# wuji3/visiondk

Hardware: AMD Instinct MI355X
Metric: images/sec fwd+bwd+optimizer step (ViT-B/16, bs=256 per GPU) (higher is better)
Workload: dtype fp16; 1 GPU; ViT-B/16 ICT, synthetic ImageNet-1k 224x224, random-init weights (reference re-init), per-GPU batch 256, CE label_smoothing 0.05, SGD 0.006/0.937/5e-4, clip 10, EMA on rank 0; global_batch=256, parallelism=dp1

## Files before the change

visiondk_amd/csrc/vit_engine.hip:

```cpp
#include <hip/hip_runtime.h>
#include <stdlib.h>
#include <stdio.h>
#include <string.h>
#include "vdk_device.h"
#include "vdk_host.h"
#include "vdk_gemm.h"

extern "C" {
int vdk_layernorm_fwd(const float*, int64_t, int32_t, int32_t, const float*, const float*, float, void*, int64_t, int32_t, float*, float*, void*);
int vdk_layernorm_bwd_workspace_bytes(int32_t, int32_t, size_t*);
int vdk_layernorm_bwd(const void*, int64_t, int32_t, const float*, int64_t, const float*, const float*, const float*, const float*, int64_t,
                      int32_t, int32_t, float*, int64_t, void*, int64_t, float*, float*, void*, size_t, void*);
int vdk_reduce_rows_f32(const float*, int64_t, int32_t, int64_t, float*, float, void*);
int vdk_colsum_bf16_workspace_bytes(int32_t, int32_t, size_t*);
int vdk_colsum_bf16(const void*, int64_t, int32_t, int32_t, float*, void*, size_t, void*);
int vdk_attention_fwd(const void*, int64_t, void*, int64_t, float*, int32_t, int32_t, int32_t, int32_t, float, void*);
int vdk_attention_bwd(const void*, int64_t, const void*, const void*, int64_t, const float*, void*, int64_t, float*, int32_t, int32_t, int32_t,
                      int32_t, float, void*);
int vdk_attention_fwd_dt(const void*, int64_t, void*, int64_t, float*, int32_t, int32_t, int32_t, int32_t, float, int32_t, void*);
int vdk_attention_bwd_dt(const void*, int64_t, const void*, const void*, int64_t, const float*, void*, int64_t, float*, int32_t, int32_t, int32_t, int32_t, float, int32_t, void*);
int vdk_attention_bwd_cs(const void*, int64_t, const void*, const void*, int64_t, const float*, void*, int64_t, float*, int32_t, int32_t, int32_t, int32_t, float, int32_t, float*, int32_t*,
                         void*);
int vdk_patchify_bf16(const float*, int32_t, int32_t, int32_t, int32_t, int32_t, void*, int32_t, void*);
int vdk_cls_rows(float*, int64_t, int32_t, int32_t, const float*, const float*, void*);
// ... 161 lines not shown
  size_t dxa, dxm;
  size_t dxab[3], dxmb[2];
  size_t du[2], dqkv[2];
  size_t dsm;
  size_t dvec;
  size_t tA, tB;
  size_t slabs, slabs_bytes;
  size_t lnws, lnws_bytes, csws, csws_bytes;
  size_t dhf;
  size_t dposall;
  size_t a8;
  size_t a8b;
};
static size_t w_take(size_t& cur, size_t n) { size_t o = cur; cur = (cur + n + 255) & ~(size_t)255; return o; }
static int wgrad_splitk(int M, int N, int K) {
  if (K < 4096) return 1;
  int tiles = ((M + 127) / 128) * ((N + 127) / 128);
  int s = (1024 + tiles - 1) / tiles;
  if (s > 32) s = 32;
  if (s < 1) s = 1;
  return s;
}
static int wgrad_splitk_tn(int M, int N, int K) {
  const int tiles = ((M + 255) / 256) * ((N + 255) / 256);
  int s = 256 / tiles;
  if (s < 1) s = 1;
  const int kt = K / 64;
  if (s > kt / 4) s = kt / 4;
  if (s > 64) s = 64;
  if (s < 1) s = 1;
  return s;
}
static int vit_plan(const VitDims& d, WsPlan* w) {
  size_t cur = 0;
  const size_t T = d.T, D = d.D, M = d.M, L = d.L;
  w->patches = w_take(cur, (size_t)d.B * d.np * d.Kpe * 2);
  w->pepad = w->dwpe = 0;
  if (d.Kraw != d.Kpe) { w->pepad = w_take(cur, D * d.Kpe * 2); w->dwpe = w_take(cur, D * d.Kpe * 4); }
  w->X = w_take(cur, (2 * L + 1) * T * D * 4);
  w->xe = w->pstats = 0;
  if (d.pre) { w->xe = w_take(cur, T * D * 4); w->pstats = w_take(cur, 2 * T * 4); }
  w->stats = w_take(cur, (L * 4 * T + 2 * T) * 4);
  w->s_h = T * D * 2; w->s_qkv = T * 3 * D * 2; w->s_lse = (size_t)d.B * d.H * d.N * 4; w->s_u = T * M * 2;
  w->h1 = w_take(cur, L * w->s_h); w->qkv = w_take(cur, L * w->s_qkv); w->lse = w_take(cur, L * w->s_lse);
  w->o = w_take(cur, L * w->s_h); w->h2 = w_take(cur, L * w->s_h); w->u = w_take(cur, L * w->s_u); w->g = w_take(cur, L * w->s_u);
  w->hf = w_take(cur, (size_t)d.Bp * D * 2);
  w->dxa = w_take(cur, T * D * 4); w->dxm = w_take(cur, T * D * 4);
  size_t big = M > 3 * D ? M : 3 * D;
  for (int i = 0; i < 3; ++i) w->dxab[i] = w_take(cur, T * D * 2);
  for (int i = 0; i < 2; ++i) {
    w->dxmb[i] = w_take(cur, T * D * 2);
    w->du[i] = w_take(cur, T * M * 2); w->dqkv[i] = w_take(cur, T * 3 * D * 2);
  }
  w->dsm = w_take(cur, T * D * 2);
  w->dvec = w_take(cur, w->s_lse);
  size_t trows = big > (size_t)d.Cp ? big : (size_t)d.Cp;
  if (trows < (size_t)d.Kpe) trows = d.Kpe;
  size_t tcols = d.Tp > d.Bp ? d.Tp : d.Bp;
  w->tA = w_take(cur, trows * tcols * 2); w->tB = w_take(cur, trows * tcols * 2);
  size_t sl = 0;
  {
    int sh[5][3] = {{(int)M, (int)D, d.T}, {(int)D, (int)M, d.T}, {3 * (int)D, (int)D, d.T}, {(int)D, (int)D, d.T}, {(int)D, d.Kpe, d.B * d.np}};
    for (auto& s : sh) {
      int k1 = wgrad_splitk(s[0], s[1], s[2]), k2 = wgrad_splitk_tn(s[0], s[1], s[2]);
      size_t b = (size_t)(k1 > k2 ? k1 : k2) * s[0] * s[1] * 4; if (b > sl) sl = b;
    }
  }
  w->slabs_bytes = sl; w->slabs = w_take(cur, sl);
  vdk_layernorm_bwd_workspace_bytes(d.T, d.D, &w->lnws_bytes); w->lnws_bytes = (w->lnws_bytes + 255) & ~(size_t)255; w->lnws = w_take(cur, 2 * w->lnws_bytes);
  size_t cs = (size_t)((tcols + 63) / 64) * trows * 4;
  { size_t cs2 = 0; vdk_colsum_bf16_workspace_bytes(d.T, (int)trows, &cs2); if (cs2 > cs) cs = cs2; }
  { size_t cs3 = (size_t)2 * ((d.T + 255) / 256) * trows * 4; if (cs3 > cs) cs = cs3; }
  w->csws_bytes = (cs + 255) & ~(size_t)255; w->csws = w_take(cur, 5 * w->csws_bytes);
  w->dhf = w_take(cur, (size_t)d.B * D * 2);
  w->dposall = w_take(cur, (size_t)d.N * D * 4);
  w->a8 = d.fp8 ? w_take(cur, T * (M > 3 * D ? M : 3 * D)) : 0;
  w->a8b = d.fp8 ? w_take(cur, T * M) : 0;
  w->total = cur;
  return VDK_OK;
}

#define RC(x) do { int rc_ = (x); if (rc_) return rc_; } while (0)

struct F8 {
  int mode; unsigned char* w8; unsigned char* wt8; float* amax; float* sc; float* si; unsigned char* a8; unsigned char* a8b;
};
static int f8_init(const VdkVitConfig* cfg, const VitDims& d, const PLayout& p, F8* f, unsigned char* a8, unsigned char* a8b) {
  f->mode = d.fp8; f->a8 = a8; f->a8b = a8b;
  if (!d.fp8) return VDK_OK;
  if (!cfg->fp8_w || !cfg->fp8_state) return vdk_fail(VDK_EINVAL, "vit: fp8 mode without fp8_w / fp8_state");
  if (a8 && d.T < 256) return vdk_fail(VDK_EUNSUPPORTED, "vit: the fp8 mode needs batch * tokens >= 256");
  f->w8 = (unsigned char*)cfg->fp8_w; f->wt8 = f->w8 + p.total;
  const int S = 12 * d.L;
  f->amax = cfg->fp8_state; f->sc = f->amax + S; f->si = f->sc + S;
  return VDK_OK;
}
static int f8_quant(hipStream_t s, const F8& f, const void* x, int xdt, long n, int slot, int fmt, unsigned char* out, int force_current = 0) {
  if (f.mode == 2 || force_current) {
    RC(vdk_quant_fp8(x, xdt, n, nullptr, nullptr, fmt, f.amax + slot, s));
    RC(vdk_fp8_scale_update(f.amax + slot, f.sc + slot, f.si + slot, 1, fmt, 1.0f, s));
  }
  return vdk_quant_fp8(x, xdt, n, f.sc + slot, out, fmt, f.amax + slot, s);
}
static bool f8_fused(const F8& f) {
  const char* e = getenv("VDK_FP8_FUSED_QUANT");
  return f.mode == 1 && !(e && e[0] == '0');
}
static int gemm8(hipStream_t s, const F8& f, const void* a, int slot_a, int a_fmt, const unsigned char* w8, int slot_w, int64_t ldb, void* Cc, int64_t ldc, int M, int N,
                 int K, int cdt, const float* bias, const float* res, int64_t ldr, int act, void* aux, int64_t ldaux, const unsigned char* a_pre = nullptr, int q8_slot = -1,
                 int q8_fmt = 0, float* c_colsum = nullptr) {
  if (!a_pre) RC(f8_quant(s, f, a, VDK_BF16, (long)M * K, slot_a, a_fmt, f.a8));
  VdkGemmDesc g = {};
  g.A = a_pre ? a_pre : f.a8; g.lda = K; g.B = w8; g.ldb = ldb; g.C = Cc; g.ldc = ldc; g.M = M; g.N = N; g.K = K; g.c_dtype = cdt; g.bias = bias; g.residual = res; g.ldr = ldr;
  g.act = act; g.aux = aux; g.ldaux = ldaux; g.alpha = 1.0f; g.splitk = 1; g.c_colsum = c_colsum;
  if (q8_slot >= 0) return vdk_gemm_fp8_nt_q8(&g, a_fmt, 0, f.si + slot_a, f.si + slot_w, f.a8b, N, q8_fmt, f.sc + q8_slot, f.amax + q8_slot, s);
  return vdk_gemm_fp8_nt(&g, a_fmt, 0, f.si + slot_a, f.si + slot_w, s);
}
__global__ void vit_fp8_update_kernel(float* __restrict__ amax, float* __restrict__ sc, float* __restrict__ si, int n) {
  const int i = blockIdx.x * blockDim.x + threadIdx.x;
  if (i >= n) return;
  const float a = amax[i], fmax = (i % 12) >= 8 ? 57344.0f : 448.0f;
  if (a > 0.f && a < 3.0e38f) { const float v = fmax / a; sc[i] = v; si[i] = 1.0f / v; }
  amax[i] = 0.f;
}

#include <map>
#include <vector>
static thread_local std::map<int, std::vector<hipEvent_t>> g_ev_dev;
static int ev_get(size_t i, hipEvent_t* e) {
  int dev = 0; (void)hipGetDevice(&dev);
  std::vector<hipEvent_t>& g_ev = g_ev_dev[dev];
  while (g_ev.size() <= i) {
    hipEvent_t x;
    if (hipEventCreateWithFlags(&x, hipEventDisableTiming) != hipSuccess) return vdk_fail(VDK_ELAUNCH, "vit: hipEventCreate failed");
    g_ev.push_back(x);
  }
  *e = g_ev[i];
  return VDK_OK;
}
static int ev_order(size_t slot, hipStream_t from, hipStream_t to) {
  if (from == to) return VDK_OK;
  hipEvent_t e; RC(ev_get(slot, &e));
  if (hipEventRecord(e, from) != hipSuccess || hipStreamWaitEvent(to, e, 0) != hipSuccess) return vdk_fail(VDK_ELAUNCH, "vit: event record/wait failed");
  return VDK_OK;
}

static int gemm(hipStream_t s, const void* A, int64_t lda, const void* B, int64_t ldb, void* C, int64_t ldc, int M, int N, int K, int cdt,
                const float* bias, const float* res, int64_t ldr, int act, void* aux, int64_t ldaux, int splitk, int row_group, void* ws,
                size_t wsb) {
  VdkGemmDesc g = {};
  g.A = A; g.lda = lda; g.B = B; g.ldb = ldb; g.C = C; g.ldc = ldc; g.M = M; g.N = N; g.K = K; g.c_dtype = cdt == VDK_F32 ? VDK_F32 : DT16; g.bias = bias;
  g.residual = res; g.ldr = ldr; g.act = act; g.aux = aux; g.ldaux = ldaux; g.alpha = 1.0f; g.splitk = splitk; g.row_group = row_group; g.ab_dtype = DT16;
  return vdk_gemm_bf16_nt(&g, ws, wsb, s);
}

extern "C" {

int vdk_vit_param_count(const VdkVitConfig* cfg, int64_t* n_floats, int32_t* n_tensors, int64_t* n_transposed) {
  VitDims d; RC(vit_dims(cfg, &d));
  PLayout p; RC(vit_layout(d, &p));
  if (n_floats) *n_floats = p.total;
  if (n_tensors) *n_tensors = 3 + d.pre + d.cls + 12 * d.L + (d.C > 0 ? 4 : 2);
  if (n_transposed) *n_transposed = p.totalT;
  return VDK_OK;
}

// ... 15 lines not shown
  VitDims d; RC(vit_dims(cfg, &d));
  WsPlan w; RC(vit_plan(d, &w));
  if (!bytes) return vdk_fail(VDK_EINVAL, "null");
  *bytes = w.total;
  return VDK_OK;
}

int vdk_vit_refresh_weights(const VdkVitConfig* cfg, const float* params, void* wb16, void* wt16, int32_t skip_wb16, void* stream) {
  VitDims d; RC(vit_dims(cfg, &d));
  PLayout p; RC(vit_layout(d, &p));
  if (!params || !wb16 || !wt16) return vdk_fail(VDK_EINVAL, "vdk_vit_refresh_weights: null pointer");
  t_opf = d.opf;
  if (!skip_wb16) RC(vdk_cast_f32_16(params, wb16, p.total, t_opf, stream));
  bf16_t* wt = (bf16_t*)wt16;
  std::vector<VdkTcItem> jobs;
  auto add = [&](const float* in, int ldi, int R, int Cc, bf16_t* out, int ldo, int Rpad) { jobs.push_back(VdkTcItem{in, out, ldi, R, Cc, ldo, Rpad}); };
  for (int l = 0; l < d.L; ++l) {
    add(params + p.blk[l].qkv_w, d.D, 3 * d.D, d.D, wt + p.blkT[l].qkv, 3 * d.D, 3 * d.D);
    add(params + p.blk[l].proj_w, d.D, d.D, d.D, wt + p.blkT[l].proj, d.D, d.D);
    add(params + p.blk[l].fc1_w, d.D, d.M, d.D, wt + p.blkT[l].fc1, d.M, d.M);
    add(params + p.blk[l].fc2_w, d.M, d.D, d.M, wt + p.blkT[l].fc2, d.D, d.D);
  }
  if (d.C > 0) add(params + p.head_w, d.D, d.Cp, d.D, wt + p.headT, d.Cp, d.Cp);
  RC(vdk_transpose_cast_batch(jobs.data(), (int)jobs.size(), stream, t_opf));
  if (d.fp8) {
    F8 f; RC(f8_init(cfg, d, p, &f, nullptr, nullptr));
    hipStream_t s = (hipStream_t)stream;
    for (int l = 0; l < d.L; ++l) {
      const PLayout::Blk& b = p.blk[l]; const PLayout::BlkT& bt = p.blkT[l];
      const int64_t off[4] = {b.qkv_w, b.proj_w, b.fc1_w, b.fc2_w}, offT[4] = {bt.qkv, bt.proj, bt.fc1, bt.fc2};
      const long n[4] = {(long)3 * d.D * d.D, (long)d.D * d.D, (long)d.M * d.D, (long)d.D * d.M};
      for (int k = 0; k < 4; ++k) {
        RC(f8_quant(s, f, params + off[k], VDK_F32, n[k], 12 * l + 4 + k, 0, f.w8 + off[k], 1));
        RC(vdk_quant_fp8(wt + offT[k], VDK_BF16, n[k], f.sc + 12 * l + 4 + k, f.wt8 + offT[k], 0, nullptr, s));
      }
    }
  }
  return VDK_OK;
}

int vdk_vit_fp8_update(const VdkVitConfig* cfg, void* stream) {
  VitDims d; RC(vit_dims(cfg, &d));
  if (!d.fp8) return VDK_OK;
  if (!cfg->fp8_state) return vdk_fail(VDK_EINVAL, "vdk_vit_fp8_update: null state");
  const int S = 12 * d.L;
  hipLaunchKernelGGL(vit_fp8_update_kernel, dim3((unsigned)((S + 255) / 256)), dim3(256), 0, (hipStream_t)stream, cfg->fp8_state, cfg->fp8_state + S, cfg->fp8_state + 2 * S, S);
  return vdk_check_launch("vdk_vit_fp8_update");
}

int vdk_vit_forward(const VdkVitConfig* cfg, const float* x, const float* params, const void* wb16, void* ws, size_t ws_bytes,
                    float* logits, void* stream_) {
  hipStream_t s = (hipStream_t)stream_;
  VitDims d; RC(vit_dims(cfg, &d));
  PLayout p; RC(vit_layout(d, &p));
  WsPlan w; RC(vit_plan(d, &w));
  if (!x || !params || !wb16 || !ws || !logits) return vdk_fail(VDK_EINVAL, "vdk_vit_forward: null pointer");
  if (ws_bytes < w.total) return vdk_fail(VDK_EWORKSPACE, "vdk_vit_forward: workspace too small");
  t_opf = d.opf;
  char* base = (char*)ws;
  const bf16_t* wb = (const bf16_t*)wb16;
  const int T = d.T, D = d.D, M = d.M;
  float* X = (float*)(base + w.X);
  float* stats = (float*)(base + w.stats);
  const size_t XS = (size_t)T * D;

  bf16_t* patches = (bf16_t*)(base + w.patches);
  RC(vdk_patchify_16(x, d.B, d.Cin, d.img, d.img, d.ps, patches, d.Kpe, t_opf, s));
  const bf16_t* pew = wb + p.pe_w;
  if (d.Kraw != d.Kpe) {
    RC(vdk_cast_pad_rows(params + p.pe_w, d.Kraw, D, d.Kraw, base + w.pepad, d.Kpe, s, t_opf));
    pew = (const bf16_t*)(base + w.pepad);
  }
  float* const X0 = d.pre ? (float*)(base + w.xe) : X;
  RC(gemm(s, patches, d.Kpe, pew, d.Kpe, X0, D, d.B * d.np, D, d.Kpe, VDK_F32, params + p.pe_b, params + p.pos, D, VDK_ACT_NONE,
          nullptr, 0, 1, d.cls ? d.np : -d.np, nullptr, 0));
  if (d.cls) RC(vdk_cls_rows(X0, (int64_t)d.N * D, d.B, D, params + p.cls, params + p.pos, s));
  if (d.pre) {
    float* ps = (float*)(base + w.pstats);
    RC(vdk_layernorm_fwd(X0, D, T, D, params + p.npre_w, params + p.npre_b, d.eps, X, D, VDK_F32, ps, ps + T, s));
  }

  const float scale = 0.125f;
  F8 f8; RC(f8_init(cfg, d, p, &f8, (unsigned char*)(base + w.a8), (unsigned char*)(base + w.a8b)));
  for (int l = 0; l < d.L; ++l) {
    const PLayout::Blk& b = p.blk[l];
    float* xin = X + (size_t)(2 * l) * XS; float* xmid = xin + XS; float* xout = xmid + XS;
    float* mean1 = stats + (size_t)l * 4 * T; float* rstd1 = mean1 + T; float* mean2 = rstd1 + T; float* rstd2 = mean2 + T;
    bf16_t* h1 = (bf16_t*)(base + w.h1 + l * w.s_h); bf16_t* qkv = (bf16_t*)(base + w.qkv + l * w.s_qkv);
    float* lse = (float*)(base + w.lse + l * w.s_lse); bf16_t* o = (bf16_t*)(base + w.o + l * w.s_h);
    bf16_t* h2 = (bf16_t*)(base + w.h2 + l * w.s_h); bf16_t* u = (bf16_t*)(base + w.u + l * w.s_u); bf16_t* g = (bf16_t*)(base + w.g + l * w.s_u);
    if (f8.mode) {
      const int sl = 12 * l;
      const bool fl = f8_fused(f8) && D > 128 && D <= 1024, fq = f8_fused(f8) && (M % 64) == 0;
      if (fl) RC(vdk_layernorm_fwd_q8(xin, D, T, D, params + b.n1w, params + b.n1b, d.eps, h1, D, mean1, rstd1, f8.a8, D, 0, f8.sc + sl + 0, f8.amax + sl + 0, s));
      else RC(vdk_layernorm_fwd(xin, D, T, D, params + b.n1w, params + b.n1b, d.eps, h1, D, VDK_BF16, mean1, rstd1, s));
      RC(gemm8(s, f8, h1, sl + 0, 0, f8.w8 + b.qkv_w, sl + 4, D, qkv, 3 * D, T, 3 * D, D, VDK_BF16, params + b.qkv_b, nullptr, 0, VDK_ACT_NONE, nullptr, 0, fl ? f8.a8 : nullptr));
      RC(vdk_attention_fwd(qkv, 3 * D, o, D, lse, d.B, d.N, d.H, 64, scale, s));
      RC(gemm8(s, f8, o, sl + 1, 0, f8.w8 + b.proj_w, sl + 5, D, xmid, D, T, D, D, VDK_F32, params + b.proj_b, xin, D, VDK_ACT_NONE, nullptr, 0));
      if (fl) RC(vdk_layernorm_fwd_q8(xmid, D, T, D, params + b.n2w, params + b.n2b, d.eps, h2, D, mean2, rstd2, f8.a8, D, 0, f8.sc + sl + 2, f8.amax + sl + 2, s));
      else RC(vdk_layernorm_fwd(xmid, D, T, D, params + b.n2w, params + b.n2b, d.eps, h2, D, VDK_BF16, mean2, rstd2, s));
      RC(gemm8(s, f8, h2, sl + 2, 0, f8.w8 + b.fc1_w, sl + 6, D, g, M, T, M, D, VDK_BF16, params + b.fc1_b, nullptr, 0, VDK_ACT_GELU, u, M, fl ? f8.a8 : nullptr, fq ? sl + 3 : -1, 0));
      RC(gemm8(s, f8, g, sl + 3, 0, f8.w8 + b.fc2_w, sl + 7, M, xout, D, T, D, M, VDK_F32, params + b.fc2_b, xmid, D, VDK_ACT_NONE, nullptr, 0, fq ? f8.a8b : nullptr));
      continue;
    }
    RC(vdk_layernorm_fwd(xin, D, T, D, params + b.n1w, params + b.n1b, d.eps, h1, D, DT16, mean1, rstd1, s));
    RC(gemm(s, h1, D, wb + b.qkv_w, D, qkv, 3 * D, T, 3 * D, D, DT16, params + b.qkv_b, nullptr, 0, VDK_ACT_NONE, nullptr, 0, 1, 0, nullptr, 0));
    RC(vdk_attention_fwd_dt(qkv, 3 * D, o, D, lse, d.B, d.N, d.H, 64, scale, DT16, s));
    RC(gemm(s, o, D, wb + b.proj_w, D, xmid, D, T, D, D, VDK_F32, params + b.proj_b, xin, D, VDK_ACT_NONE, nullptr, 0, 1, 0, nullptr, 0));
    RC(vdk_layernorm_fwd(xmid, D, T, D, params + b.n2w, params + b.n2b, d.eps, h2, D, DT16, mean2, rstd2, s));
    RC(gemm(s, h2, D, wb + b.fc1_w, D, g, M, T, M, D, DT16, params + b.fc1_b, nullptr, 0, ACT_FC1, u, M, 1, 0, nullptr, 0));
    RC(gemm(s, g, M, wb + b.fc2_w, M, xout, D, T, D, M, VDK_F32, params + b.fc2_b, xmid, D, VDK_ACT_NONE, nullptr, 0, 1, 0, nullptr, 0));
  }
  float* xl = X + (size_t)(2 * d.L) * XS;
  float* meanf = stats + (size_t)d.L * 4 * T; float* rstdf = meanf + T;
  if (d.C == 0) {
    RC(vdk_layernorm_fwd(xl, D, T, D, params + p.norm_w, params + p.norm_b, d.eps, logits, D, VDK_F32, meanf, rstdf, s));
    return VDK_OK;
  }
  bf16_t* hf = (bf16_t*)(base + w.hf);
  RC(vdk_layernorm_fwd(xl, (int64_t)d.N * D, d.B, D, params + p.norm_w, params + p.norm_b, d.eps, hf, D, DT16, meanf, rstdf, s));
  RC(gemm(s, hf, D, wb + p.head_w, D, logits, d.Cp, d.B, d.Cp, D, VDK_F32, params + p.head_b, nullptr, 0, VDK_ACT_NONE, nullptr, 0, 1, 0, nullptr, 0));
  return VDK_OK;
}

static int linear_wgrad(hipStream_t s, const VitDims& d, const WsPlan& w, char* base, const bf16_t* dY, int64_t lddy, const bf16_t* Xa,
                        int64_t ldx, int rows, int rows_pad, int out, int in, float* dW, float* db, int dy_row_group) {
  if ((rows % 64) == 0 && (out % 8) == 0 && (in % 8) == 0 && out >= 8 && in >= 8 && !(t_opf && dy_row_group != 0)) {
    const int sk = wgrad_splitk_tn(out, in, rows);
    VdkGemmDesc g = {};
    g.A = dY; g.lda = lddy; g.B = Xa; g.ldb = ldx; g.C = dW; g.ldc = in; g.M = out; g.N = in; g.K = rows; g.c_dtype = VDK_F32;
    g.alpha = 1.0f; g.splitk = sk; g.trans = 1; g.a_row_group = dy_row_group; g.ab_dtype = DT16;
    RC(vdk_gemm_bf16_nt(&g, base + w.slabs, w.slabs_bytes, s));
    if (db && dy_row_group == 0) RC(vdk_colsum_16(dY, lddy, rows, out, db, base + w.csws + 4 * w.csws_bytes, w.csws_bytes, t_opf, s));
    return VDK_OK;
  }
  bf16_t* tA = (bf16_t*)(base + w.tA); bf16_t* tB = (bf16_t*)(base + w.tB);
  float* csp = (db && dy_row_group == 0) ? (float*)(base + w.csws + 4 * w.csws_bytes) : nullptr;
  RC(vdk_transpose_16(dY, lddy, rows, out, tA, rows_pad, rows_pad, dy_row_group, csp, t_opf, s));
  RC(vdk_transpose_16(Xa, ldx, rows, in, tB, rows_pad, rows_pad, 0, nullptr, t_opf, s));
  const int sk = wgrad_splitk(out, in, rows_pad);
  RC(gemm(s, tA, rows_pad, tB, rows_pad, dW, in, out, in, rows_pad, VDK_F32, nullptr, nullptr, 0, VDK_ACT_NONE, nullptr, 0, sk, 0, base + w.slabs,
          w.slabs_bytes));
  if (csp) RC(vdk_reduce_rows_f32(csp, out, (rows_pad + 63) / 64, out, db, 1.0f, s));
  return VDK_OK;
}

static bool qkvb_pass(int T, int N, size_t csws_bytes) {
  static const int env = getenv("VDK_VIT_QKVB_PASS") ? atoi(getenv("VDK_VIT_QKVB_PASS")) : -1;
  if (env == 0) return false;
  size_t need = 0;
  if (vdk_colsum_bf16_workspace_bytes(T, N, &need) != VDK_OK || need > csws_bytes) return false;
  return true;
}

static int dgrad_with_bias(hipStream_t s, const WsPlan& w, char* base, const bf16_t* dY, int64_t lddy, const bf16_t* Wt, int64_t ldw, void* dX, int64_t lddx, int rows,
                           int in, int out, int act, void* aux, int64_t ldaux, float* db, int* fused, int slot, VdkReduceJob* jobs, int* njobs,
                           float* dbx = nullptr, int* fusedx = nullptr, int slotx = 0) {
  const int prow = db ? vdk_gemm_a_colsum_rows(rows, in, out) : 0;
  *fused = (db && !t_opf && prow > 0 && (size_t)prow * out * 4 <= w.csws_bytes) ? 1 : 0;
  const int xrow = dbx ? vdk_gemm_c_colsum_rows(rows, in, out) : 0;
  const int fx = (dbx && !*fused && xrow > 0 && (size_t)xrow * in * 4 <= w.csws_bytes) ? 1 : 0;
  if (fusedx) *fusedx = fx;
  float* const part = (float*)(base + w.csws + (size_t)slot * w.csws_bytes);
  float* const partx = (float*)(base + w.csws + (size_t)slotx * w.csws_bytes);
  VdkGemmDesc g = {};
  g.A = dY; g.lda = lddy; g.B = Wt; g.ldb = ldw; g.C = dX; g.ldc = lddx; g.M = rows; g.N = in; g.K = out; g.c_dtype = DT16; g.act = act; g.aux = aux;
  g.ldaux = ldaux; g.alpha = 1.0f; g.splitk = 1; g.ab_dtype = DT16;
  if (*fused) g.a_colsum = part;
  if (fx) g.c_colsum = partx;
  RC(vdk_gemm_bf16_nt(&g, nullptr, 0, s));
  if (*fused) jobs[(*njobs)++] = VdkReduceJob{part, (long)out, prow, (long)out, db, 1.0f};
  if (fx) jobs[(*njobs)++] = VdkReduceJob{partx, (long)in, xrow, (long)in, dbx, 1.0f};
  return VDK_OK;
}

int vdk_vit_backward(const VdkVitConfig* cfg, const void* dlogits, const float* params, const void* wb16, const void* wt16, void* ws,
                     size_t ws_bytes, float* grads, vdk_grad_ready_fn on_ready, void* user, void* stream_, void* side_stream_) {
  hipStream_t s = (hipStream_t)stream_;
  hipStream_t s2 = side_stream_ ? (hipStream_t)side_stream_ : s;
  VitDims d; RC(vit_dims(cfg, &d));
  PLayout p; RC(vit_layout(d, &p));
  WsPlan w; RC(vit_plan(d, &w));
  if (!dlogits || !params || !wb16 || !wt16 || !ws || !grads) return vdk_fail(VDK_EINVAL, "vdk_vit_backward: null pointer");
  if (ws_bytes < w.total) return vdk_fail(VDK_EWORKSPACE, "vdk_vit_backward: workspace too small");
  t_opf = d.opf;
  char* base = (char*)ws;
  const bf16_t* wt = (const bf16_t*)wt16;
  const int T = d.T, D = d.D, M = d.M;
  float* X = (float*)(base + w.X);
  float* stats = (float*)(base + w.stats);
  const size_t XS = (size_t)T * D;
  float* dxa = (float*)(base + w.dxa); float* dxm = (float*)(base + w.dxm);
#define DXAB(l) ((bf16_t*)(base + w.dxab[((l) + 3) % 3]))
#define DXMB(l) ((bf16_t*)(base + w.dxmb[((l) + 2) & 1]))
#define DU(l) ((bf16_t*)(base + w.du[((l) + 2) & 1]))
#define DQKV(l) ((bf16_t*)(base + w.dqkv[((l) + 2) & 1]))
  bf16_t* dsm = (bf16_t*)(base + w.dsm);
  float* dvec = (float*)(base + w.dvec);
  void* lnws = base + w.lnws;
  const size_t EV_SIDE_DONE = 8;
  size_t ev_p = EV_SIDE_DONE + d.L + 4;
  RC(ev_order(0, s, s2));

  bool last_fc2_bias_done = false;
  if (d.C == 0) {
    float* xl = X + (size_t)(2 * d.L) * XS;
    float* meanf = stats + (size_t)d.L * 4 * T; float* rstdf = meanf + T;
    RC(vdk_layernorm_bwd_deferred(dlogits, D, VDK_F32, xl, D, meanf, rstdf, params + p.norm_w, nullptr, 0, T, D, dxa, D, DXAB(d.L - 1), D, grads + p.norm_w,
                                  grads + p.norm_b, lnws, w.lnws_bytes, s, nullptr, nullptr, nullptr, nullptr, t_opf));
    if (on_ready) on_ready(user, p.norm_w, p.total - p.norm_w);
  } else {
    const bf16_t* dl = (const bf16_t*)dlogits;
    bf16_t* hf = (bf16_t*)(base + w.hf);
    RC(linear_wgrad(s, d, w, base, dl, d.Cp, hf, D, d.B, d.Bp, d.Cp, D, grads + p.head_w, grads + p.head_b, 0));
    bf16_t* dhf = (bf16_t*)(base + w.dhf);
    RC(gemm(s, dl, d.Cp, wt + p.headT, d.Cp, dhf, D, d.B, D, d.Cp, DT16, nullptr, nullptr, 0, VDK_ACT_NONE, nullptr, 0, 1, 0, nullptr, 0));
    if (hipMemsetAsync(dxa, 0, XS * 4, s) != hipSuccess || hipMemsetAsync(DXAB(d.L - 1), 0, XS * 2, s) != hipSuccess)
      return vdk_fail(VDK_ELAUNCH, "vdk_vit_backward: memset failed");
    float* xl = X + (size_t)(2 * d.L) * XS;
    float* meanf = stats + (size_t)d.L * 4 * T; float* rstdf = meanf + T;
    if (s2 == s && D <= 1024) {
      VdkReduceJob fj[2];
      RC(vdk_layernorm_bwd_deferred(dhf, D, DT16, xl, (int64_t)d.N * D, meanf, rstdf, params + p.norm_w, nullptr, 0, d.B, D, dxa, (int64_t)d.N * D, DXAB(d.L - 1),
                                    (int64_t)d.N * D, grads + p.norm_w, grads + p.norm_b, lnws, w.lnws_bytes, s, &fj[0], grads + p.blk[d.L - 1].fc2_b, &fj[1]));
      if (fj[0].in) RC(vdk_reduce_rows_batch(fj, 2, s)); else RC(vdk_reduce_rows_batch(fj + 1, 1, s));
      last_fc2_bias_done = true;
    } else
    RC(vdk_layernorm_bwd(dhf, D, DT16, xl, (int64_t)d.N * D, meanf, rstdf, params + p.norm_w, nullptr, 0, d.B, D, dxa, (int64_t)d.N * D, DXAB(d.L - 1),
                         (int64_t)d.N * D, grads + p.norm_w, grads + p.norm_b, lnws, w.lnws_bytes, s));
    if (on_ready) on_ready(user, p.norm_w, p.total - p.norm_w);
  }
  bool fc2_bias_from_norm1 = false, dxab8_ready = false;
  F8 f8; RC(f8_init(cfg, d, p, &f8, (unsigned char*)(base + w.a8), (unsigned char*)(base + w.a8b)));
  for (int l = d.L - 1; l >= 0; --l) {
    const PLayout::Blk& b = p.blk[l];
    float* xin = X + (size_t)(2 * l) * XS; float* xmid = xin + XS;
    float* mean1 = stats + (size_t)l * 4 * T; float* rstd1 = mean1 + T; float* mean2 = rstd1 + T; float* rstd2 = mean2 + T;
    bf16_t* h1 = (bf16_t*)(base + w.h1 + l * w.s_h); bf16_t* qkv = (bf16_t*)(base + w.qkv + l * w.s_qkv);
    float* lse = (float*)(base + w.lse + l * w.s_lse); bf16_t* o = (bf16_t*)(base + w.o + l * w.s_h);
    bf16_t* h2 = (bf16_t*)(base + w.h2 + l * w.s_h); bf16_t* u = (bf16_t*)(base + w.u + l * w.s_u); bf16_t* g = (bf16_t*)(base + w.g + l * w.s_u);
    bf16_t* dxab = DXAB(l); bf16_t* dxmb = DXMB(l); bf16_t* du = DU(l); bf16_t* dqkv = DQKV(l);
    if (s2 != s && l + 2 <= d.L - 1) { hipEvent_t e; RC(ev_get(EV_SIDE_DONE + l + 3, &e)); if (hipStreamWaitEvent(s, e, 0) != hipSuccess) return vdk_fail(VDK_ELAUNCH, "vit: wait failed"); }
    int fz = 0;
    const bool one_stream = (s2 == s);
    VdkReduceJob jobs[8]; int nj = 0;
    char* const lnws0 = base + w.lnws; char* const lnws1 = lnws0 + w.lnws_bytes;
    RC(ev_order(ev_p++, s, s2));
    if (f8.mode) {
      const int sl = 12 * l;
      const bool have_fc2b = one_stream && ((l == d.L - 1) ? last_fc2_bias_done : fc2_bias_from_norm1);
      const bool fq = f8_fused(f8) && (M % 64) == 0;
      const int xrow = one_stream ? 2 * ((T + 255) / 256) : 0;
      const bool fo = xrow > 0 && (size_t)xrow * M * 4 <= w.csws_bytes;
      float* const partx = (float*)(base + w.csws + (size_t)1 * w.csws_bytes);
      RC(gemm8(s, f8, dxab, sl + 8, 1, f8.wt8 + p.blkT[l].fc2, sl + 7, D, du, M, T, M, D, VDK_BF16, nullptr, nullptr, 0, VDK_ACT_DGELU, u, M, dxab8_ready ? f8.a8 : nullptr,
               fq ? sl + 9 : -1, 1, fo ? partx : nullptr));
      if (fo) jobs[nj++] = VdkReduceJob{partx, (long)M, xrow, (long)M, grads + b.fc1_b, 1.0f};
      RC(linear_wgrad(s2, d, w, base, dxab, D, g, M, T, d.Tp, D, M, grads + b.fc2_w, have_fc2b ? nullptr : grads + b.fc2_b, 0));
      RC(gemm8(s, f8, du, sl + 9, 1, f8.wt8 + p.blkT[l].fc1, sl + 6, M, dsm, D, T, D, M, VDK_BF16, nullptr, nullptr, 0, VDK_ACT_NONE, nullptr, 0, fq ? f8.a8b : nullptr));
      RC(linear_wgrad(s2, d, w, base, du, M, h2, D, T, d.Tp, M, D, grads + b.fc1_w, fo ? nullptr : grads + b.fc1_b, 0));
    } else if (one_stream) {
      int fx = 0;
      const bool have_fc2b = (l == d.L - 1) ? last_fc2_bias_done : fc2_bias_from_norm1;
      RC(dgrad_with_bias(s, w, base, dxab, D, wt + p.blkT[l].fc2, D, du, M, T, M, D, ACT_DFC2, u, M, have_fc2b ? nullptr : grads + b.fc2_b, &fz, 0, jobs, &nj,
                         grads + b.fc1_b, &fx, 1));
      RC(linear_wgrad(s2, d, w, base, dxab, D, g, M, T, d.Tp, D, M, grads + b.fc2_w, (fz || have_fc2b) ? nullptr : grads + b.fc2_b, 0));
      if (fx) {
        RC(gemm(s, du, M, wt + p.blkT[l].fc1, M, dsm, D, T, D, M, DT16, nullptr, nullptr, 0, VDK_ACT_NONE, nullptr, 0, 1, 0, nullptr, 0));
        fz = 1;
      } else {
        RC(dgrad_with_bias(s, w, base, du, M, wt + p.blkT[l].fc1, M, dsm, D, T, D, M, VDK_ACT_NONE, nullptr, 0, grads + b.fc1_b, &fz, 1, jobs, &nj));
      }
      RC(linear_wgrad(s2, d, w, base, du, M, h2, D, T, d.Tp, M, D, grads + b.fc1_w, fz ? nullptr : grads + b.fc1_b, 0));
    } else {
      RC(linear_wgrad(s2, d, w, base, dxab, D, g, M, T, d.Tp, D, M, grads + b.fc2_w, grads + b.fc2_b, 0));
      RC(gemm(s, dxab, D, wt + p.blkT[l].fc2, D, du, M, T, M, D, DT16, nullptr, nullptr, 0, ACT_DFC2, u, M, 1, 0, nullptr, 0));
      RC(ev_order(ev_p++, s, s2));
      RC(linear_wgrad(s2, d, w, base, du, M, h2, D, T, d.Tp, M, D, grads + b.fc1_w, grads + b.fc1_b, 0));
      RC(gemm(s, du, M, wt + p.blkT[l].fc1, M, dsm, D, T, D, M, DT16, nullptr, nullptr, 0, VDK_ACT_NONE, nullptr, 0, 1, 0, nullptr, 0));
    }
    const bool ocs_ln = one_stream && D <= 1024;
    static const bool g16_on = !(getenv("VDK_VIT_G16") && atoi(getenv("VDK_VIT_G16")) == 0);
    const bool g16 = g16_on && ocs_ln && !f8.mode && t_opf == VDK_OPF_F16 && D > 512 && D <= 1024;
    const bool lq = f8.mode && f8_fused(f8) && ocs_ln;
    const LnQ8 q8m = {f8.a8, (long)D, f8.sc + 12 * l + 10, f8.amax + 12 * l + 10, 1};
    if (g16) RC(vdk_layernorm_bwd_deferred(dsm, D, DT16, xmid, D, mean2, rstd2, params + b.n2w, nullptr, D, T, D, nullptr, D, dxmb, D, grads + b.n2w, grads + b.n2b, lnws0,
                                           w.lnws_bytes, s, &jobs[nj], grads + b.proj_b, &jobs[nj + 1], nullptr, 0, nullptr, nullptr, 1, dxab));
    else
    RC(vdk_layernorm_bwd_deferred(dsm, D, DT16, xmid, D, mean2, rstd2, params + b.n2w, dxa, D, T, D, dxm, D, dxmb, D, grads + b.n2w, grads + b.n2b, lnws0,
                                  w.lnws_bytes, s, &jobs[nj], ocs_ln ? grads + b.proj_b : nullptr, ocs_ln ? &jobs[nj + 1] : nullptr, lq ? &q8m : nullptr));
    nj += ocs_ln ? 2 : 1;
    RC(ev_order(ev_p++, s, s2));
    if (f8.mode) {
      RC(gemm8(s, f8, dxmb, 12 * l + 10, 1, f8.wt8 + p.blkT[l].proj, 12 * l + 5, D, dsm, D, T, D, D, VDK_BF16, nullptr, nullptr, 0, VDK_ACT_NONE, nullptr, 0, lq ? f8.a8 : nullptr));
      RC(linear_wgrad(s2, d, w, base, dxmb, D, o, D, T, d.Tp, D, D, grads + b.proj_w, ocs_ln ? nullptr : grads + b.proj_b, 0));
    } else if (one_stream && ocs_ln) {
      RC(gemm(s, dxmb, D, wt + p.blkT[l].proj, D, dsm, D, T, D, D, DT16, nullptr, nullptr, 0, VDK_ACT_NONE, nullptr, 0, 1, 0, nullptr, 0));
      RC(linear_wgrad(s2, d, w, base, dxmb, D, o, D, T, d.Tp, D, D, grads + b.proj_w, nullptr, 0));
    } else if (one_stream) {
      RC(dgrad_with_bias(s, w, base, dxmb, D, wt + p.blkT[l].proj, D, dsm, D, T, D, D, VDK_ACT_NONE, nullptr, 0, grads + b.proj_b, &fz, 2, jobs, &nj));
      RC(linear_wgrad(s2, d, w, base, dxmb, D, o, D, T, d.Tp, D, D, grads + b.proj_w, fz ? nullptr : grads + b.proj_b, 0));
    } else {
      RC(linear_wgrad(s2, d, w, base, dxmb, D, o, D, T, d.Tp, D, D, grads + b.proj_w, grads + b.proj_b, 0));
      RC(gemm(s, dxmb, D, wt + p.blkT[l].proj, D, dsm, D, T, D, D, DT16, nullptr, nullptr, 0, VDK_ACT_NONE, nullptr, 0, 1, 0, nullptr, 0));
    }
    int32_t qkvb_done = 0;
    {
      static const bool fuse_on = !(getenv("VDK_VIT_QKVB_ATTN") && atoi(getenv("VDK_VIT_QKVB_ATTN")) == 0);
      float* csp = (fuse_on && !f8.mode && one_stream && (size_t)d.B * 3 * D * 4 <= w.csws_bytes) ? (float*)(base + w.csws + (size_t)3 * w.csws_bytes) : nullptr;
      RC(vdk_attention_bwd_cs(qkv, 3 * D, o, dsm, D, lse, dqkv, 3 * D, dvec, d.B, d.N, d.H, 64, 0.125f, DT16, csp, &qkvb_done, s));
      if (qkvb_done) { jobs[nj] = VdkReduceJob{csp, (long)3 * D, d.B, (long)3 * D, grads + b.qkv_b, 1.0f}; ++nj; }
    }
    RC(ev_order(ev_p++, s, s2));
    if (f8.mode) {
      size_t csneed = 0; vdk_colsum_bf16_workspace_bytes(T, 3 * D, &csneed);
      const bool fcq = f8_fused(f8) && one_stream && csneed <= w.csws_bytes;
      if (fcq) {
        const LnQ8 q8d = {f8.a8, (long)3 * D, f8.sc + 12 * l + 11, f8.amax + 12 * l + 11, 1};
        RC(vdk_colsum_bf16_deferred(dqkv, 3 * D, T, 3 * D, grads + b.qkv_b, base + w.csws + (size_t)2 * w.csws_bytes, w.csws_bytes, s, &jobs[nj], &q8d)); ++nj;
      }
      RC(gemm8(s, f8, dqkv, 12 * l + 11, 1, f8.wt8 + p.blkT[l].qkv, 12 * l + 4, 3 * D, dsm, D, T, D, 3 * D, VDK_BF16, nullptr, nullptr, 0, VDK_ACT_NONE, nullptr, 0,
               fcq ? f8.a8 : nullptr));
      RC(linear_wgrad(s2, d, w, base, dqkv, 3 * D, h1, D, T, d.Tp, 3 * D, D, grads + b.qkv_w, fcq ? nullptr : grads + b.qkv_b, 0));
    } else if (one_stream && (qkvb_done || qkvb_pass(T, 3 * D, w.csws_bytes))) {
      if (!qkvb_done) { RC(vdk_colsum_bf16_deferred(dqkv, 3 * D, T, 3 * D, grads + b.qkv_b, base + w.csws + (size_t)3 * w.csws_bytes, w.csws_bytes, s, &jobs[nj], nullptr, t_opf)); ++nj; }
      RC(gemm(s, dqkv, 3 * D, wt + p.blkT[l].qkv, 3 * D, dsm, D, T, D, 3 * D, DT16, nullptr, nullptr, 0, VDK_ACT_NONE, nullptr, 0, 1, 0, nullptr, 0));
      RC(linear_wgrad(s2, d, w, base, dqkv, 3 * D, h1, D, T, d.Tp, 3 * D, D, grads + b.qkv_w, nullptr, 0));
    } else if (one_stream) {
      RC(dgrad_with_bias(s, w, base, dqkv, 3 * D, wt + p.blkT[l].qkv, 3 * D, dsm, D, T, D, 3 * D, VDK_ACT_NONE, nullptr, 0, grads + b.qkv_b, &fz, 3, jobs, &nj));
      RC(linear_wgrad(s2, d, w, base, dqkv, 3 * D, h1, D, T, d.Tp, 3 * D, D, grads + b.qkv_w, fz ? nullptr : grads + b.qkv_b, 0));
    } else {
      RC(linear_wgrad(s2, d, w, base, dqkv, 3 * D, h1, D, T, d.Tp, 3 * D, D, grads + b.qkv_w, grads + b.qkv_b, 0));
      RC(gemm(s, dqkv, 3 * D, wt + p.blkT[l].qkv, 3 * D, dsm, D, T, D, 3 * D, DT16, nullptr, nullptr, 0, VDK_ACT_NONE, nullptr, 0, 1, 0, nullptr, 0));
    }
    const bool ocs_n1 = ocs_ln && l > 0;
    const bool lq1 = lq && ocs_n1;
    const LnQ8 q8a = {f8.a8, (long)D, f8.sc + 12 * (l - 1) + 8, f8.amax + 12 * (l - 1) + 8, 1};
    if (g16 && l > 0) RC(vdk_layernorm_bwd_deferred(dsm, D, DT16, xin, D, mean1, rstd1, params + b.n1w, nullptr, D, T, D, nullptr, D, DXAB(l - 1), D, grads + b.n1w, grads + b.n1b, lnws1,
                                                    w.lnws_bytes, s, &jobs[nj], grads + p.blk[l - 1].fc2_b, &jobs[nj + 1], nullptr, 0, nullptr, nullptr, 1, dxmb));
    else if (g16) {
      float* const dummy_cs = (float*)(base + w.csws);
      RC(vdk_layernorm_bwd_deferred(dsm, D, DT16, xin, D, mean1, rstd1, params + b.n1w, nullptr, D, T, D, dxa, D, DXAB(l - 1), D, grads + b.n1w, grads + b.n1b, lnws1,
                                    w.lnws_bytes, s, &jobs[nj], dummy_cs, &jobs[nj + 1], nullptr, 0, nullptr, nullptr, 1, dxmb));
    } else
    RC(vdk_layernorm_bwd_deferred(dsm, D, DT16, xin, D, mean1, rstd1, params + b.n1w, dxm, D, T, D, dxa, D, DXAB(l - 1), D, grads + b.n1w, grads + b.n1b, lnws1,
                                  w.lnws_bytes, s, &jobs[nj], ocs_n1 ? grads + p.blk[l - 1].fc2_b : nullptr, ocs_n1 ? &jobs[nj + 1] : nullptr, lq1 ? &q8a : nullptr));
    dxab8_ready = lq1;
    nj += ocs_n1 ? 2 : 1;
    fc2_bias_from_norm1 = ocs_n1;
    RC(vdk_reduce_rows_batch(jobs, nj, s));
    if (s2 != s) { hipEvent_t e; RC(ev_get(EV_SIDE_DONE + l + 1, &e)); if (hipEventRecord(e, s2) != hipSuccess) return vdk_fail(VDK_ELAUNCH, "vit: record failed"); }
    if (on_ready) {
      if (s2 != s) { hipEvent_t e; RC(ev_get(EV_SIDE_DONE + l + 1, &e)); if (hipStreamWaitEvent(s, e, 0) != hipSuccess) return vdk_fail(VDK_ELAUNCH, "vit: wait failed"); }
      on_ready(user, b.n1w, (l + 1 < d.L ? p.blk[l + 1].n1w : p.norm_w) - b.n1w);
    }
  }
  {
    float* dposall = (float*)(base + w.dposall);
    const float* dx0 = dxa;
    if (d.pre) {
      const float* ps = (const float*)(base + w.pstats);
      RC(vdk_layernorm_bwd_deferred(dxa, D, VDK_F32, (const float*)(base + w.xe), D, ps, ps + T, params + p.npre_w, nullptr, 0, T, D, dxm, D, DXAB(-1), D, grads + p.npre_w,
                                    grads + p.npre_b, lnws, w.lnws_bytes, s, nullptr, nullptr, nullptr, nullptr, t_opf));
      dx0 = dxm;
    }
    RC(vdk_reduce_rows_f32(dx0, (int64_t)d.N * D, d.B, (int64_t)d.N * D, grads + p.pos, 1.0f, s));
    if (d.cls && hipMemcpyAsync(grads + p.cls, grads + p.pos, (size_t)D * 4, hipMemcpyDeviceToDevice, s) != hipSuccess)
      return vdk_fail(VDK_ELAUNCH, "vdk_vit_backward: memcpy failed");
    if (!d.pre) RC(vdk_reduce_rows_f32(grads + p.pos + (size_t)d.cls * D, D, d.np, D, grads + p.pe_b, 1.0f, s));
    else if (hipMemsetAsync(grads + p.pe_b, 0, (size_t)D * 4, s) != hipSuccess) return vdk_fail(VDK_ELAUNCH, "vdk_vit_backward: memset failed");
    (void)dposall;
    bf16_t* patches = (bf16_t*)(base + w.patches);
    const int rows = d.B * d.np, rows_pad = (int)up(rows, 64);
    RC(ev_order(ev_p++, s, s2));
    float* dwpe = d.Kraw != d.Kpe ? (float*)(base + w.dwpe) : grads + p.pe_w;
    RC(linear_wgrad(s2, d, w, base, DXAB(-1), D, patches, d.Kpe, rows, rows_pad, D, d.Kpe, dwpe, nullptr, d.cls ? d.np : 0));
    if (d.Kraw != d.Kpe && hipMemcpy2DAsync(grads + p.pe_w, (size_t)d.Kraw * 4, dwpe, (size_t)d.Kpe * 4, (size_t)d.Kraw * 4, D, hipMemcpyDeviceToDevice, s2) != hipSuccess)
      return vdk_fail(VDK_ELAUNCH, "vdk_vit_backward: memcpy2d failed");
    RC(ev_order(ev_p++, s2, s));
    if (on_ready) on_ready(user, 0, p.blk[0].n1w);
  }
#undef DXAB
#undef DXMB
#undef DU
#undef DQKV
  return vdk_check_launch("vdk_vit_backward");
}
// ... 94 lines not shown
```

Before: 7385 images/sec.

## Restrict last ViT block's post-attention path to CLS token rows

When the classifier reads only the CLS token, the last transformer block's proj, LayerNorm2, MLP fc1/fc2 forward and their backward gradients are now computed for just the B CLS rows, using a strided leading dimension, instead of all T tokens. Backward zeroes the gradient buffers for the skipped rows in place of the earlier full dx memsets. This removes roughly the MLP and proj work of one of 12 blocks. It is exact because the other rows do not affect the loss, but the strided small-M GEMMs may run less efficiently. It can be turned off with VDK_VIT_CLS_TAIL=0.

New measurement: 7705 images/sec, median of 6. +4.3%, better.

```diff
diff --git a/visiondk_amd/csrc/vit_engine.hip b/visiondk_amd/csrc/vit_engine.hip
--- a/visiondk_amd/csrc/vit_engine.hip
+++ b/visiondk_amd/csrc/vit_engine.hip
@@ -267,6 +267,11 @@
 
 #define RC(x) do { int rc_ = (x); if (rc_) return rc_; } while (0)
 
+static bool cls_tail_on(const VitDims& d) {
+  const char* e = getenv("VDK_VIT_CLS_TAIL");
+  return d.C > 0 && d.cls && !d.fp8 && !(e && e[0] == '0');
+}
+
 struct F8 {
   int mode; unsigned char* w8; unsigned char* wt8; float* amax; float* sc; float* si; unsigned char* a8; unsigned char* a8b;
 };
@@ -448,6 +453,7 @@
 
   const float scale = 0.125f;
   F8 f8; RC(f8_init(cfg, d, p, &f8, (unsigned char*)(base + w.a8), (unsigned char*)(base + w.a8b)));
+  const bool cls_tail = cls_tail_on(d);
   for (int l = 0; l < d.L; ++l) {
     const PLayout::Blk& b = p.blk[l];
     float* xin = X + (size_t)(2 * l) * XS; float* xmid = xin + XS; float* xout = xmid + XS;
@@ -472,10 +478,13 @@
     RC(vdk_layernorm_fwd(xin, D, T, D, params + b.n1w, params + b.n1b, d.eps, h1, D, DT16, mean1, rstd1, s));
     RC(gemm(s, h1, D, wb + b.qkv_w, D, qkv, 3 * D, T, 3 * D, D, DT16, params + b.qkv_b, nullptr, 0, VDK_ACT_NONE, nullptr, 0, 1, 0, nullptr, 0));
     RC(vdk_attention_fwd_dt(qkv, 3 * D, o, D, lse, d.B, d.N, d.H, 64, scale, DT16, s));
-    RC(gemm(s, o, D, wb + b.proj_w, D, xmid, D, T, D, D, VDK_F32, params + b.proj_b, xin, D, VDK_ACT_NONE, nullptr, 0, 1, 0, nullptr, 0));
-    RC(vdk_layernorm_fwd(xmid, D, T, D, params + b.n2w, params + b.n2b, d.eps, h2, D, DT16, mean2, rstd2, s));
-    RC(gemm(s, h2, D, wb + b.fc1_w, D, g, M, T, M, D, DT16, params + b.fc1_b, nullptr, 0, ACT_FC1, u, M, 1, 0, nullptr, 0));
-    RC(gemm(s, g, M, wb + b.fc2_w, M, xout, D, T, D, M, VDK_F32, params + b.fc2_b, xmid, D, VDK_ACT_NONE, nullptr, 0, 1, 0, nullptr, 0));
+    const bool tail = cls_tail && l == d.L - 1;
+    const int R = tail ? d.B : T;
+    const int64_t ldt = tail ? (int64_t)d.N * D : D;
+    RC(gemm(s, o, ldt, wb + b.proj_w, D, xmid, ldt, R, D, D, VDK_F32, params + b.proj_b, xin, ldt, VDK_ACT_NONE, nullptr, 0, 1, 0, nullptr, 0));
+    RC(vdk_layernorm_fwd(xmid, ldt, R, D, params + b.n2w, params + b.n2b, d.eps, h2, D, DT16, mean2, rstd2, s));
+    RC(gemm(s, h2, D, wb + b.fc1_w, D, g, M, R, M, D, DT16, params + b.fc1_b, nullptr, 0, ACT_FC1, u, M, 1, 0, nullptr, 0));
+    RC(gemm(s, g, M, wb + b.fc2_w, M, xout, ldt, R, D, M, VDK_F32, params + b.fc2_b, xmid, ldt, VDK_ACT_NONE, nullptr, 0, 1, 0, nullptr, 0));
   }
   float* xl = X + (size_t)(2 * d.L) * XS;
   float* meanf = stats + (size_t)d.L * 4 * T; float* rstdf = meanf + T;
@@ -567,6 +576,7 @@
   const size_t EV_SIDE_DONE = 8;
   size_t ev_p = EV_SIDE_DONE + d.L + 4;
   RC(ev_order(0, s, s2));
+  const bool cls_tail = cls_tail_on(d);
 
   bool last_fc2_bias_done = false;
   if (d.C == 0) {
@@ -581,7 +591,7 @@
     RC(linear_wgrad(s, d, w, base, dl, d.Cp, hf, D, d.B, d.Bp, d.Cp, D, grads + p.head_w, grads + p.head_b, 0));
     bf16_t* dhf = (bf16_t*)(base + w.dhf);
     RC(gemm(s, dl, d.Cp, wt + p.headT, d.Cp, dhf, D, d.B, D, d.Cp, DT16, nullptr, nullptr, 0, VDK_ACT_NONE, nullptr, 0, 1, 0, nullptr, 0));
-    if (hipMemsetAsync(dxa, 0, XS * 4, s) != hipSuccess || hipMemsetAsync(DXAB(d.L - 1), 0, XS * 2, s) != hipSuccess)
+    if (!cls_tail && (hipMemsetAsync(dxa, 0, XS * 4, s) != hipSuccess || hipMemsetAsync(DXAB(d.L - 1), 0, XS * 2, s) != hipSuccess))
       return vdk_fail(VDK_ELAUNCH, "vdk_vit_backward: memset failed");
     float* xl = X + (size_t)(2 * d.L) * XS;
     float* meanf = stats + (size_t)d.L * 4 * T; float* rstdf = meanf + T;
@@ -611,6 +621,14 @@
     const bool one_stream = (s2 == s);
     VdkReduceJob jobs[8]; int nj = 0;
     char* const lnws0 = base + w.lnws; char* const lnws1 = lnws0 + w.lnws_bytes;
+    const bool ocs_ln = one_stream && D <= 1024;
+    static const bool g16_on = !(getenv("VDK_VIT_G16") && atoi(getenv("VDK_VIT_G16")) == 0);
+    const bool g16 = g16_on && ocs_ln && !f8.mode && t_opf == VDK_OPF_F16 && D > 512 && D <= 1024;
+    const bool tail = cls_tail && l == d.L - 1;
+    const int R = tail ? d.B : T, Rp = tail ? d.Bp : d.Tp;
+    const int64_t ldt = tail ? (int64_t)d.N * D : D;
+    if (tail && (hipMemsetAsync(dsm, 0, XS * 2, s) != hipSuccess || (g16 ? hipMemsetAsync(dxmb, 0, XS * 2, s) : hipMemsetAsync(dxm, 0, XS * 4, s)) != hipSuccess))
+      return vdk_fail(VDK_ELAUNCH, "vdk_vit_backward: memset failed");
     RC(ev_order(ev_p++, s, s2));
     if (f8.mode) {
       const int sl = 12 * l;
@@ -628,32 +646,29 @@
     } else if (one_stream) {
       int fx = 0;
       const bool have_fc2b = (l == d.L - 1) ? last_fc2_bias_done : fc2_bias_from_norm1;
-      RC(dgrad_with_bias(s, w, base, dxab, D, wt + p.blkT[l].fc2, D, du, M, T, M, D, ACT_DFC2, u, M, have_fc2b ? nullptr : grads + b.fc2_b, &fz, 0, jobs, &nj,
+      RC(dgrad_with_bias(s, w, base, dxab, ldt, wt + p.blkT[l].fc2, D, du, M, R, M, D, ACT_DFC2, u, M, have_fc2b ? nullptr : grads + b.fc2_b, &fz, 0, jobs, &nj,
                          grads + b.fc1_b, &fx, 1));
-      RC(linear_wgrad(s2, d, w, base, dxab, D, g, M, T, d.Tp, D, M, grads + b.fc2_w, (fz || have_fc2b) ? nullptr : grads + b.fc2_b, 0));
+      RC(linear_wgrad(s2, d, w, base, dxab, ldt, g, M, R, Rp, D, M, grads + b.fc2_w, (fz || have_fc2b) ? nullptr : grads + b.fc2_b, 0));
       if (fx) {
-        RC(gemm(s, du, M, wt + p.blkT[l].fc1, M, dsm, D, T, D, M, DT16, nullptr, nullptr, 0, VDK_ACT_NONE, nullptr, 0, 1, 0, nullptr, 0));
+        RC(gemm(s, du, M, wt + p.blkT[l].fc1, M, dsm, ldt, R, D, M, DT16, nullptr, nullptr, 0, VDK_ACT_NONE, nullptr, 0, 1, 0, nullptr, 0));
         fz = 1;
       } else {
-        RC(dgrad_with_bias(s, w, base, du, M, wt + p.blkT[l].fc1, M, dsm, D, T, D, M, VDK_ACT_NONE, nullptr, 0, grads + b.fc1_b, &fz, 1, jobs, &nj));
+        RC(dgrad_with_bias(s, w, base, du, M, wt + p.blkT[l].fc1, M, dsm, ldt, R, D, M, VDK_ACT_NONE, nullptr, 0, grads + b.fc1_b, &fz, 1, jobs, &nj));
       }
-      RC(linear_wgrad(s2, d, w, base, du, M, h2, D, T, d.Tp, M, D, grads + b.fc1_w, fz ? nullptr : grads + b.fc1_b, 0));
+      RC(linear_wgrad(s2, d, w, base, du, M, h2, D, R, Rp, M, D, grads + b.fc1_w, fz ? nullptr : grads + b.fc1_b, 0));
     } else {
-      RC(linear_wgrad(s2, d, w, base, dxab, D, g, M, T, d.Tp, D, M, grads + b.fc2_w, grads + b.fc2_b, 0));
-      RC(gemm(s, dxab, D, wt + p.blkT[l].fc2, D, du, M, T, M, D, DT16, nullptr, nullptr, 0, ACT_DFC2, u, M, 1, 0, nullptr, 0));
+      RC(linear_wgrad(s2, d, w, base, dxab, ldt, g, M, R, Rp, D, M, grads + b.fc2_w, grads + b.fc2_b, 0));
+      RC(gemm(s, dxab, ldt, wt + p.blkT[l].fc2, D, du, M, R, M, D, DT16, nullptr, nullptr, 0, ACT_DFC2, u, M, 1, 0, nullptr, 0));
       RC(ev_order(ev_p++, s, s2));
-      RC(linear_wgrad(s2, d, w, base, du, M, h2, D, T, d.Tp, M, D, grads + b.fc1_w, grads + b.fc1_b, 0));
-      RC(gemm(s, du, M, wt + p.blkT[l].fc1, M, dsm, D, T, D, M, DT16, nullptr, nullptr, 0, VDK_ACT_NONE, nullptr, 0, 1, 0, nullptr, 0));
-    }
-    const bool ocs_ln = one_stream && D <= 1024;
-    static const bool g16_on = !(getenv("VDK_VIT_G16") && atoi(getenv("VDK_VIT_G16")) == 0);
-    const bool g16 = g16_on && ocs_ln && !f8.mode && t_opf == VDK_OPF_F16 && D > 512 && D <= 1024;
+      RC(linear_wgrad(s2, d, w, base, du, M, h2, D, R, Rp, M, D, grads + b.fc1_w, grads + b.fc1_b, 0));
+      RC(gemm(s, du, M, wt + p.blkT[l].fc1, M, dsm, ldt, R, D, M, DT16, nullptr, nullptr, 0, VDK_ACT_NONE, nullptr, 0, 1, 0, nullptr, 0));
+    }
     const bool lq = f8.mode && f8_fused(f8) && ocs_ln;
     const LnQ8 q8m = {f8.a8, (long)D, f8.sc + 12 * l + 10, f8.amax + 12 * l + 10, 1};
-    if (g16) RC(vdk_layernorm_bwd_deferred(dsm, D, DT16, xmid, D, mean2, rstd2, params + b.n2w, nullptr, D, T, D, nullptr, D, dxmb, D, grads + b.n2w, grads + b.n2b, lnws0,
+    if (g16) RC(vdk_layernorm_bwd_deferred(dsm, ldt, DT16, xmid, ldt, mean2, rstd2, params + b.n2w, nullptr, ldt, R, D, nullptr, ldt, dxmb, ldt, grads + b.n2w, grads + b.n2b, lnws0,
                                            w.lnws_bytes, s, &jobs[nj], grads + b.proj_b, &jobs[nj + 1], nullptr, 0, nullptr, nullptr, 1, dxab));
     else
-    RC(vdk_layernorm_bwd_deferred(dsm, D, DT16, xmid, D, mean2, rstd2, params + b.n2w, dxa, D, T, D, dxm, D, dxmb, D, grads + b.n2w, grads + b.n2b, lnws0,
+    RC(vdk_layernorm_bwd_deferred(dsm, ldt, DT16, xmid, ldt, mean2, rstd2, params + b.n2w, dxa, ldt, R, D, dxm, ldt, dxmb, ldt, grads + b.n2w, grads + b.n2b, lnws0,
                                   w.lnws_bytes, s, &jobs[nj], ocs_ln ? grads + b.proj_b : nullptr, ocs_ln ? &jobs[nj + 1] : nullptr, lq ? &q8m : nullptr));
     nj += ocs_ln ? 2 : 1;
     RC(ev_order(ev_p++, s, s2));
@@ -661,14 +676,14 @@
       RC(gemm8(s, f8, dxmb, 12 * l + 10, 1, f8.wt8 + p.blkT[l].proj, 12 * l + 5, D, dsm, D, T, D, D, VDK_BF16, nullptr, nullptr, 0, VDK_ACT_NONE, nullptr, 0, lq ? f8.a8 : nullptr));
       RC(linear_wgrad(s2, d, w, base, dxmb, D, o, D, T, d.Tp, D, D, grads + b.proj_w, ocs_ln ? nullptr : grads + b.proj_b, 0));
     } else if (one_stream && ocs_ln) {
-      RC(gemm(s, dxmb, D, wt + p.blkT[l].proj, D, dsm, D, T, D, D, DT16, nullptr, nullptr, 0, VDK_ACT_NONE, nullptr, 0, 1, 0, nullptr, 0));
-      RC(linear_wgrad(s2, d, w, base, dxmb, D, o, D, T, d.Tp, D, D, grads + b.proj_w, nullptr, 0));
+      RC(gemm(s, dxmb, ldt, wt + p.blkT[l].proj, D, dsm, ldt, R, D, D, DT16, nullptr, nullptr, 0, VDK_ACT_NONE, nullptr, 0, 1, 0, nullptr, 0));
+      RC(linear_wgrad(s2, d, w, base, dxmb, ldt, o, ldt, R, Rp, D, D, grads + b.proj_w, nullptr, 0));
     } else if (one_stream) {
-      RC(dgrad_with_bias(s, w, base, dxmb, D, wt + p.blkT[l].proj, D, dsm, D, T, D, D, VDK_ACT_NONE, nullptr, 0, grads + b.proj_b, &fz, 2, jobs, &nj));
-      RC(linear_wgrad(s2, d, w, base, dxmb, D, o, D, T, d.Tp, D, D, grads + b.proj_w, fz ? nullptr : grads + b.proj_b, 0));
+      RC(dgrad_with_bias(s, w, base, dxmb, ldt, wt + p.blkT[l].proj, D, dsm, ldt, R, D, D, VDK_ACT_NONE, nullptr, 0, grads + b.proj_b, &fz, 2, jobs, &nj));
+      RC(linear_wgrad(s2, d, w, base, dxmb, ldt, o, ldt, R, Rp, D, D, grads + b.proj_w, fz ? nullptr : grads + b.proj_b, 0));
     } else {
-      RC(linear_wgrad(s2, d, w, base, dxmb, D, o, D, T, d.Tp, D, D, grads + b.proj_w, grads + b.proj_b, 0));
-      RC(gemm(s, dxmb, D, wt + p.blkT[l].proj, D, dsm, D, T, D, D, DT16, nullptr, nullptr, 0, VDK_ACT_NONE, nullptr, 0, 1, 0, nullptr, 0));
+      RC(linear_wgrad(s2, d, w, base, dxmb, ldt, o, ldt, R, Rp, D, D, grads + b.proj_w, grads + b.proj_b, 0));
+      RC(gemm(s, dxmb, ldt, wt + p.blkT[l].proj, D, dsm, ldt, R, D, D, DT16, nullptr, nullptr, 0, VDK_ACT_NONE, nullptr, 0, 1, 0, nullptr, 0));
     }
     int32_t qkvb_done = 0;
     {
```
